# bit-current/DistributedTraining

Measured on AMD Instinct MI355X. Metric: tokens/sec (whole node, all miners), GPT-2-small local-SGD, higher is better.
Workload: dtype bf16; 1 GPU; model=gpt2-small, global_batch=1024, seq_len=64, parallelism=local_sgd_dp1, merge_every=25, optimizer=fused AdamW (lr 5e-4, reference config)

## Files before the change

### distributedtraining_amd/ops/__init__.py

```python

from __future__ import annotations

import math
from typing import Optional

import torch
import torch.nn.functional as F

from . import droprng
from .backend import require_ext, use_hip

__all__ = [
    "layer_norm", "rms_norm", "gelu", "swiglu", "causal_attention",
    "qkv_attention", "linear", "mlp_gelu", "add_layer_norm",
    "add_rms_norm",
    "cross_entropy_loss", "lm_head_ce", "lm_head_loss",
    "embedding_fwd",
    "decode_attention", "rope", "adamw_step", "delta_sub", "axpy_",
    "weighted_merge",
    "grad_merge_weights", "has_nan", "l2norm",
    "quantize_blockwise_int8", "dequantize_blockwise_int8",
    "dropout", "rng_tick",
]

# ... 22 lines not shown
        if dy2.stride(-1) != 1:
            dy2 = dy2.contiguous()
        dx = dy2.mm(w).view(ctx.xshape)
        m = require_ext()
        if _USE_BGRADB and ctx.has_b and ctx.wgrad is not None:
            try:
                db = m.lt_wgrad_bgradb(dy2, x2, ctx.wgrad)
                return dx, None, db
            except RuntimeError:
                pass
        if ctx.wgrad is not None:
            ctx.wgrad.addmm_(dy2.t(), x2)
            dw = None
        else:
            dw = dy2.t().mm(x2)
        db = (_grad_out(m.colsum(dy2), ctx.bgrad, w.dtype)
              if ctx.has_b else None)
        return dx, dw, db


def linear(x: torch.Tensor, w: torch.Tensor,
           b: Optional[torch.Tensor] = None) -> torch.Tensor:
    if use_hip(x):
        rows = x.numel() // x.shape[-1]
        if rows <= 4 and not torch.is_grad_enabled() and _gemv_wins(rows, w):
            x2 = x.reshape(rows, x.shape[-1])
            if not x2.is_contiguous():
                x2 = x2.contiguous()
            y = require_ext().gemv(
                x2, w, b if b is not None
                else torch.empty(0, dtype=w.dtype, device=w.device))
# ... 22 lines not shown
        y = torch.addmm(b2, h, w2.t())
        ctx.save_for_backward(x2, w1, w2, h, aux)
        ctx.xshape = x.shape
        ctx.w1grad = getattr(w1, "main_grad", None)
        ctx.w2grad = getattr(w2, "main_grad", None)
        ctx.b2grad = getattr(b2, "main_grad", None)
        return y.view(*x.shape[:-1], w2.shape[0])

    @staticmethod
    def backward(ctx, dy):
        m = require_ext()
        x2, w1, w2, h, aux = ctx.saved_tensors
        dy2 = dy.reshape(-1, dy.shape[-1])
        if dy2.stride(-1) != 1:
            dy2 = dy2.contiguous()
        db2 = _grad_out(m.colsum(dy2), ctx.b2grad, w2.dtype)
        if ctx.w2grad is not None:
            ctx.w2grad.addmm_(dy2.t(), h)
            dw2 = None
        else:
            dw2 = dy2.t().mm(h)
        dh_pre, db1 = m.lt_dgrad_dgelu_bgrad(dy2, w2, aux)
        if ctx.w1grad is not None:
            ctx.w1grad.addmm_(dh_pre.t(), x2)
            dw1 = None
        else:
            dw1 = dh_pre.t().mm(x2)
        dx = dh_pre.mm(w1).view(ctx.xshape)
        return dx, dw1, db1, dw2, db2


def mlp_gelu(x: torch.Tensor, w1: torch.Tensor, b1: torch.Tensor,
             w2: torch.Tensor, b2: torch.Tensor) -> torch.Tensor:
    if use_hip(x):
        rows = x.numel() // x.shape[-1]
        if rows <= 4 and not torch.is_grad_enabled():
            return linear(gelu(linear(x, w1, b1)), w2, b2)
        key = (rows, w1.shape[0], w1.shape[1])
        if _lt_fused_shape_ok.get(key, True):
            try:
                out = _FusedMLPFn.apply(x, w1, b1, w2, b2)
                _lt_fused_shape_ok[key] = True
                return out
            except RuntimeError as e:
                import logging
                logging.getLogger(__name__).warning(
                    "hipBLASLt epilogue MLP unavailable at M,N,K=%s (%s); "
                    "composed path", key, e)
                _lt_fused_shape_ok[key] = False
        return linear(gelu(linear(x, w1, b1)), w2, b2)
    return F.linear(F.gelu(F.linear(x, w1, b1), approximate="tanh"), w2, b2)


def _empty_like0(t):
    return t.new_empty(0)


def _rng0(t: torch.Tensor) -> torch.Tensor:
    return droprng.counter(t.device)


def _grad_out(fp32_grad, main_grad, dtype):
    if main_grad is not None:
        require_ext().accum_f32_into_bf16(main_grad, fp32_grad)
        return None
    return fp32_grad.to(dtype)


def _cpu_drop(t: torch.Tensor, p: float, site: int) -> torch.Tensor:
    keep = droprng.elem_keep_mask(t.numel(), droprng.value(t.device), site, p)
    mask = torch.from_numpy(keep.astype("float32")).reshape(t.shape)
    return t * (mask * droprng.inv_keep(p)).to(t.dtype)


def _norm_fwd(x2, res, w, b, eps, site, p):
    m = require_ext()
    if b is None:
        y, rstd, s = m.rmsnorm_fwd(x2, res, w, eps, _rng0(x2), site, p)
        return y, (rstd,), s
    y, mean, rstd, s = m.layernorm_fwd(x2, res, w, b, eps, _rng0(x2), site, p)
    return y, (mean, rstd), s


def _norm_bwd(dy, ds, x2, w, stats, site, p):
    m = require_ext()
    if len(stats) == 1:
        dx, dw32, dres = m.rmsnorm_bwd(dy, ds, x2, w, *stats, _rng0(x2),
                                       site, p)
        return dx, dw32, None, dres
    return m.layernorm_bwd(dy, ds, x2, w, *stats, _rng0(x2), site, p)


class _NormFn(torch.autograd.Function):
    @staticmethod
    def forward(ctx, x, w, b, eps):
        x2 = x.contiguous()
        y, stats, _ = _norm_fwd(x2.view(-1, x2.shape[-1]), _empty_like0(x2),
                                w, b, eps, 0, 0.0)
        ctx.save_for_backward(x2, w, *stats)
        ctx.wg = getattr(w, "main_grad", None)
        ctx.bg = getattr(b, "main_grad", None)
        return y.view_as(x2)

    @staticmethod
    def backward(ctx, dy):
        x, w, *stats = ctx.saved_tensors
        N = x.shape[-1]
        dx, dw32, db32, _ = _norm_bwd(dy.contiguous().view(-1, N),
                                      _empty_like0(x), x.view(-1, N), w,
                                      stats, 0, 0.0)
        return (dx.view_as(x), _grad_out(dw32, ctx.wg, w.dtype),
                None if db32 is None else _grad_out(db32, ctx.bg, w.dtype),
                None)


def layer_norm(x: torch.Tensor, w: torch.Tensor, b: torch.Tensor,
               eps: float = 1e-5) -> torch.Tensor:
    if use_hip(x):
        return _NormFn.apply(x, w, b, eps)
    return F.layer_norm(x, (x.shape[-1],), w, b, eps)


class _AddNormFn(torch.autograd.Function):

    @staticmethod
    def forward(ctx, x, res, w, b, eps, p_drop, site):
        x2 = x.contiguous().view(-1, x.shape[-1])
        r2 = res.contiguous().view(-1, x.shape[-1])
# ... 1 lines not shown
        ctx.save_for_backward(s, w, *stats)
        ctx.shape = x.shape
        ctx.drop = (p_drop, site)
        ctx.wg = getattr(w, "main_grad", None)
        ctx.bg = getattr(b, "main_grad", None)
        return s.view(x.shape), y.view(x.shape)

    @staticmethod
    def backward(ctx, ds, dy):
        s, w, *stats = ctx.saved_tensors
        p_drop, site = ctx.drop
        N = s.shape[-1]
        ds2 = (ds.contiguous().view(-1, N) if ds is not None
               else _empty_like0(s))
        dx, dw32, db32, dres = _norm_bwd(dy.contiguous().view(-1, N), ds2, s,
                                         w, stats, site, p_drop)
        dx = dx.view(ctx.shape)
        dr = dres.view(ctx.shape) if p_drop > 0.0 else dx
        return (dx, dr, _grad_out(dw32, ctx.wg, w.dtype),
                None if db32 is None else _grad_out(db32, ctx.bg, w.dtype),
                None, None, None)


def add_layer_norm(x: torch.Tensor, res: torch.Tensor, w: torch.Tensor,
                   b: torch.Tensor, eps: float = 1e-5, p_drop: float = 0.0,
                   site: int = 0):
    if use_hip(x):
        return _AddNormFn.apply(x, res, w, b, eps, p_drop, site)
    if p_drop > 0.0:
        res = _cpu_drop(res, p_drop, site)
    s = x + res
    return s, F.layer_norm(s, (s.shape[-1],), w, b, eps)


def add_rms_norm(x: torch.Tensor, res: torch.Tensor, w: torch.Tensor,
# ... 696 lines not shown
```

### distributedtraining_amd/ops/hip/bindings.cpp

```cpp
#include <torch/extension.h>
#include <ATen/hip/HIPContext.h>

#include <algorithm>
#include <atomic>
#include <vector>

#include "dta_kernels.h"

namespace {

using torch::Tensor;

inline hipStream_t stream() {
  return at::hip::getCurrentHIPStream().stream();
}
inline const bf16_t* bfp(const Tensor& t) {
  return reinterpret_cast<const bf16_t*>(t.data_ptr());
}
inline bf16_t* bfp_mut(Tensor& t) {
  return reinterpret_cast<bf16_t*>(t.data_ptr());
}

void check_bf16(const Tensor& t, const char* name) {
  TORCH_CHECK(t.is_cuda(), name, " must be on GPU");
// ... 6 lines not shown
  TORCH_CHECK(t.is_contiguous(), name, " must be contiguous");
}

DropParams drop_params(const Tensor& rng, int64_t site, double p) {
  DropParams d;
  if (p > 0.0) {
    TORCH_CHECK(p < 1.0, "dropout p must be < 1");
    TORCH_CHECK(rng.numel() == 1 && rng.scalar_type() == torch::kInt64 &&
                    rng.is_cuda(), "rng must be an int64 [1] GPU counter");
    d.rng = reinterpret_cast<const unsigned long long*>(
        rng.data_ptr<int64_t>());
    d.site = (unsigned long long)site;
    dta_drop_quantize(p, d);
  }
  return d;
}

int norm_cols(const Tensor& x, int max_cols, const char* what) {
  check_bf16(x, "x");
  TORCH_CHECK(x.size(1) % 8 == 0, "cols must be a multiple of 8");
  TORCH_CHECK(x.size(1) <= max_cols, what, " supports cols <= ", max_cols,
              " (register-resident row)");
  return int(x.size(1));
}

std::vector<Tensor> norm_fwd(Tensor x, Tensor res, Tensor w, const Tensor* b,
                             double eps, Tensor rng, int64_t site, double p) {
  const int cols = norm_cols(x, DTA_NORM_FWD_MAX_COLS, "norm forward");
  check_bf16(w, "w");
  if (b) check_bf16(*b, "b");
// ... 6 lines not shown
  auto y = torch::empty_like(x);
  auto sum = has_res ? torch::empty_like(x) : torch::empty({0}, x.options());
  Tensor mean = b ? torch::empty({rows}, f32) : Tensor();
  auto rstd = torch::empty({rows}, f32);
  launch_norm_fwd({bfp(x), has_res ? bfp(res) : nullptr,
                   has_res ? bfp_mut(sum) : nullptr, bfp(w),
                   b ? bfp(*b) : nullptr, bfp_mut(y),
                   b ? mean.data_ptr<float>() : nullptr,
                   rstd.data_ptr<float>(), rows, cols, float(eps), drop, !b},
                  stream());
  return {y, mean, rstd, sum};
}

std::vector<Tensor> norm_bwd(Tensor dy, Tensor ds, Tensor x, Tensor w,
                             const Tensor* mean, Tensor rstd, Tensor rng,
                             int64_t site, double p) {
  const int cols = norm_cols(x, DTA_NORM_BWD_MAX_COLS, "norm backward");
  check_bf16(dy, "dy"); check_bf16(w, "w");
  const int64_t rows = x.size(0);
  const bool has_ds = ds.numel() > 0;
  if (has_ds) check_bf16(ds, "ds");
  const DropParams drop = drop_params(rng, site, p);
  auto dx = torch::empty_like(x);
  auto dres = drop.thr16 ? torch::empty_like(x)
                         : torch::empty({0}, x.options());
  const auto f32 = x.options().dtype(torch::kFloat32);
  auto dw32 = torch::zeros({cols}, f32);
  Tensor db32 = mean ? torch::zeros({cols}, f32) : Tensor();
  const int stripes = dta_norm_bwd_stripes(rows, cols);
  auto part = torch::empty({mean ? 2 : 1, stripes, cols}, f32);
  launch_norm_bwd({bfp(dy), has_ds ? bfp(ds) : nullptr, bfp(x), bfp(w),
                   mean ? mean->data_ptr<float>() : nullptr,
                   rstd.data_ptr<float>(), bfp_mut(dx),
                   drop.thr16 ? bfp_mut(dres) : nullptr,
                   dw32.data_ptr<float>(),
                   mean ? db32.data_ptr<float>() : nullptr,
                   part[0].data_ptr<float>(),
                   mean ? part[1].data_ptr<float>() : nullptr, stripes, rows,
                   cols, drop, !mean},
                  stream());
  return {dx, dw32, db32, dres};
}

std::vector<Tensor> layernorm_fwd(Tensor x, Tensor res, Tensor w, Tensor b,
                                  double eps, Tensor rng, int64_t site,
                                  double p) {
  return norm_fwd(x, res, w, &b, eps, rng, site, p);
}
std::vector<Tensor> layernorm_bwd(Tensor dy, Tensor ds, Tensor x, Tensor w,
                                  Tensor mean, Tensor rstd, Tensor rng,
                                  int64_t site, double p) {
  return norm_bwd(dy, ds, x, w, &mean, rstd, rng, site, p);
}
std::vector<Tensor> rmsnorm_fwd(Tensor x, Tensor res, Tensor w, double eps,
                                Tensor rng, int64_t site, double p) {
  auto o = norm_fwd(x, res, w, nullptr, eps, rng, site, p);
  return {o[0], o[2], o[3]};
}
std::vector<Tensor> rmsnorm_bwd(Tensor dy, Tensor ds, Tensor x, Tensor w,
                                Tensor rstd, Tensor rng, int64_t site,
                                double p) {
  auto o = norm_bwd(dy, ds, x, w, nullptr, rstd, rng, site, p);
  return {o[0], o[1], o[3]};
}

Tensor gelu_fwd(Tensor x) {
  auto y = torch::empty_like(x);
  if (x.scalar_type() == torch::kBFloat16) {
    check_bf16(x, "x");
    launch_gelu_fwd(bfp(x), bfp_mut(y), x.numel(), stream());
  } else {
    check_f32(x, "x");
    launch_gelu_fwd_f32(x.data_ptr<float>(), y.data_ptr<float>(), x.numel(),
                        stream());
  }
  return y;
}
// ... 79 lines not shown
  bf16_t* outp = out_bf16.numel() ? bfp_mut(out_bf16) : nullptr;
  const float* bcp = bc.numel() ? bc.data_ptr<float>() : nullptr;
  launch_adamw(master.data_ptr<float>(), grad.data_ptr(), gb,
               m.data_ptr<float>(), v.data_ptr<float>(), outp, int(step),
               bcp, float(lr), beta1, beta2, float(eps), float(wd),
               master.numel(), stream());
}

void adamw_tick(Tensor t, Tensor bc, double beta1, double beta2) {
  TORCH_CHECK(t.scalar_type() == torch::kInt32 && t.is_cuda(), "t int32 gpu");
  check_f32(bc, "bc");
  launch_adamw_tick(t.data_ptr<int>(), bc.data_ptr<float>(), beta1, beta2,
                    stream());
}

Tensor colsum(Tensor x) {
  check_bf16(x, "x");
  TORCH_CHECK(x.dim() == 2 && x.size(1) % 8 == 0,
              "x must be [rows, cols] with cols % 8 == 0");
  const int64_t rows = x.size(0);
  const int cols = int(x.size(1));
  const int stripes = dta_colred_stripes(rows, cols);
  auto f32 = x.options().dtype(torch::kFloat32);
  auto part = torch::empty({stripes, cols}, f32);
  auto out = torch::zeros({cols}, f32);
  launch_colsum(bfp(x), part.data_ptr<float>(), out.data_ptr<float>(), rows,
                cols, stripes, stream());
  return out;
}

void weighted_merge(Tensor base, Tensor deltas, Tensor W, Tensor offsets,
                    Tensor out) {
  check_f32(base, "base"); check_f32(deltas, "deltas"); check_f32(out, "out");
  auto Wc = W.to(base.device(), torch::kFloat32).contiguous();
  auto offs = offsets.to(base.device()).contiguous();
  const int n_models = int(deltas.size(0));
  const int n_segs = int(offsets.numel() - 1);
  launch_weighted_merge(base.data_ptr<float>(), deltas.data_ptr<float>(),
                        Wc.data_ptr<float>(), offs.data_ptr<int64_t>(),
                        n_models, n_segs, base.numel(),
                        out.data_ptr<float>(), stream());
}

// ... 342 lines not shown
  const int dim = int(dy.size(-1));
  const int seq = int(ids.size(-1));
  const int64_t n_tok = ids.numel();
  auto f32 = dy.options().dtype(torch::kFloat32);
  auto dwte = torch::zeros({vocab, dim}, f32);
  auto dwpe = npos ? torch::zeros({npos, dim}, f32) : torch::zeros({0}, f32);
  launch_embedding_bwd(bfp(dy), ids.data_ptr<int64_t>(),
                       dwte.data_ptr<float>(), nullptr, n_tok, seq, dim,
                       false, stream());
  if (npos) {
    const int64_t B = n_tok / seq;
    const int pcols = seq * dim;
    TORCH_CHECK(pcols % 8 == 0, "seq*dim must be a multiple of 8");
    const int stripes = dta_colred_stripes(B, pcols);
    auto part = torch::empty({stripes, pcols}, f32);
    launch_colsum(bfp(dy), part.data_ptr<float>(), dwpe.data_ptr<float>(),
                  B, pcols, stripes, stream());
  }
  return {dwte, dwpe};
}

Tensor gemv(Tensor x, Tensor w, Tensor bias) {
  check_bf16(x, "x"); check_bf16(w, "w");
  TORCH_CHECK(x.dim() == 2 && w.dim() == 2 && x.size(1) == w.size(1),
              "x [M,K], w [N,K]");
  const int M = int(x.size(0));
  TORCH_CHECK(M >= 1 && M <= 4, "gemv is for M <= 4");
  const int64_t N = w.size(0);
  const int K = int(x.size(1));
  TORCH_CHECK(K % 8 == 0, "gemv needs K % 8 == 0 (16 B row alignment)");
  const bf16_t* bp = nullptr;
  if (bias.numel()) {
// ... 205 lines not shown
}
Tensor mfma_selftest_32(Tensor A, Tensor B) {
  check_bf16(A, "A"); check_bf16(B, "B");
  auto D = torch::zeros({32, 32}, A.options().dtype(torch::kFloat32));
  launch_mfma_probe_32(bfp(A), bfp(B), D.data_ptr<float>(), stream());
  return D;
}

}

void register_lt_fused(pybind11::module& m);

PYBIND11_MODULE(TORCH_EXTENSION_NAME, m) {
  register_lt_fused(m);
  m.def("layernorm_fwd", &layernorm_fwd);
  m.def("layernorm_bwd", &layernorm_bwd);
  m.def("rmsnorm_fwd", &rmsnorm_fwd);
  m.def("rmsnorm_bwd", &rmsnorm_bwd);
  m.def("gelu_fwd", &gelu_fwd);
  m.def("gelu_bwd", &gelu_bwd);
  m.def("swiglu_fwd", &swiglu_fwd);
  m.def("swiglu_bwd", &swiglu_bwd);
  m.def("dropout_apply", &dropout_apply);
  m.def("rng_tick", &rng_tick);
  m.def("accum_f32_into_bf16", &accum_f32_into_bf16);
  m.def("delta_sub", &delta_sub);
  m.def("axpy", &axpy);
  m.def("has_nan", &has_nan);
  m.def("l2norm_sq", &l2norm_sq);
  m.def("adamw_step", &adamw_step);
  m.def("adamw_tick", &adamw_tick);
  m.def("colsum", &colsum);
  m.def("weighted_merge", &weighted_merge);
  m.def("grad_merge_weights", &grad_merge_weights);
  m.def("weighted_merge_packed", &weighted_merge_packed);
  m.def("grad_merge_weights_packed", &grad_merge_weights_packed);
  m.def("axpy_packed", &axpy_packed);
  m.def("quantize_int8", &quantize_int8);
  m.def("ce_fwd", &ce_fwd);
  m.def("ce_bwd", &ce_bwd);
  m.def("ce_fwd_bwd", &ce_fwd_bwd, pybind11::arg("logits"),
        pybind11::arg("targets"), pybind11::arg("ignore_index"),
        pybind11::arg("inv_count_dev"), pybind11::arg("max_rows") = 0,
        pybind11::arg("lds_row") = false);
  m.def("ce_chunk", &ce_chunk);
  m.def("ce_finalize", &ce_finalize);
  m.def("head_loss_fwd", &head_loss_fwd);
// ... 17 lines not shown
```

### distributedtraining_amd/ops/hip/dta_kernels.h

```cpp
#pragma once

#include <hip/hip_runtime.h>
#include <cmath>
#include <cstdint>
#include <cstdlib>

using bf16_t = unsigned short;

struct DropParams {
  const unsigned long long* rng = nullptr;
  unsigned long long site = 0;
  unsigned int thr16 = 0;
  float inv_keep = 1.0f;
};
inline void dta_drop_quantize(double p, DropParams& d) {
  const double full = 65536.0;
  d.thr16 = (unsigned int)std::fmin(std::ceil(p * full), full - 1.0);
  d.inv_keep = float(full / (full - double(d.thr16)));
}

void launch_gelu_fwd(const bf16_t* x, bf16_t* y, int64_t n, hipStream_t s);
void launch_gelu_bwd(const bf16_t* dy, const bf16_t* x, bf16_t* dx, int64_t n,
                     hipStream_t s);
void launch_gelu_fwd_f32(const float* x, float* y, int64_t n, hipStream_t s);
// ... 9 lines not shown
void launch_accum_f32_bf16(bf16_t* dst, const float* src, int64_t n,
                           hipStream_t s);

void launch_delta_sub(const float* w, const float* base, float* out,
                      int64_t n, hipStream_t s);
void launch_axpy(float* w, const float* x, float alpha, int64_t n,
                 hipStream_t s);
void launch_nan_any(const float* x, int64_t n, int* flag, hipStream_t s);
void launch_l2norm_sq(const float* x, int64_t n, float* out, hipStream_t s);
void launch_adamw(float* master, const void* grad, bool grad_is_bf16,
                  float* m, float* v, bf16_t* out_bf16, int step,
                  const float* bc_p, float lr, double beta1, double beta2,
                  float eps, float wd, int64_t n, hipStream_t s);
void launch_adamw_tick(int* t, float* bc, double beta1, double beta2,
                       hipStream_t s);
void launch_colsum(const bf16_t* x, float* part, float* out, int64_t rows,
                   int cols, int stripes, hipStream_t s);
struct ColRedCfg { int threads; int gx; int stripes; };
inline ColRedCfg dta_colred_cfg(int64_t rows, int cols) {
  const int lanes = cols / 8;
  const int gx = (lanes + 255) / 256;
  int threads = ((lanes + gx - 1) / gx + 63) / 64 * 64;
  if (threads < 64) threads = 64;
  int64_t st = (1024 * 256) / (int64_t(gx) * threads);
  const int64_t mx = (rows + 31) / 32;
  if (st > mx) st = mx;
  if (st < 1) st = 1;
  return ColRedCfg{threads, gx, int(st)};
}
inline int dta_colred_stripes(int64_t rows, int cols) {
  return dta_colred_cfg(rows, cols).stripes;
}

void launch_weighted_merge(const float* base, const float* deltas,
                           const float* W,
                           const int64_t* offsets, int n_models, int n_segs,
                           int64_t P, float* out, hipStream_t s);
void launch_grad_merge_weights(const void* g, bool g_is_bf16,
                               const float* base, const float* deltas,
                               const float* merged, const int64_t* chunks,
                               int n_models, int n_chunks, int64_t P,
                               float* grad_w,
                               int n_segs, hipStream_t s);
enum DeltaKind { DELTA_F32 = 0, DELTA_BF16 = 1, DELTA_I8 = 2 };
struct PackedView {
  const void* data;
// ... 47 lines not shown
  bf16_t* sum_out;
  const bf16_t *w, *b;
  bf16_t* y;
  float *mean, *rstd;
  int64_t rows;
  int cols;
  float eps;
  DropParams drop;
  bool rms;
};
struct NormBwdArgs {
  const bf16_t *dy, *ds, *x, *w;
  const float *mean, *rstd;
  bf16_t *dx, *dres;
  float *dw, *db, *pdw, *pdb;
  int stripes;
  int64_t rows;
  int cols;
  DropParams drop;
  bool rms;
};
void launch_norm_fwd(const NormFwdArgs& a, hipStream_t s);
void launch_norm_bwd(const NormBwdArgs& a, hipStream_t s);

void launch_ce_fwd(const bf16_t* logits, const int64_t* targets,
                   int64_t rows, int64_t vocab, int64_t ignore_index,
                   float* lse, float* loss_sum, int* count, hipStream_t s);
void launch_ce_bwd(const bf16_t* logits, const int64_t* targets,
                   const float* lse, float scale, const float* scale_p,
                   int64_t ignore_index, int64_t v0, bool nt,
// ... 106 lines not shown
```

### distributedtraining_amd/ops/hip/elementwise.hip

```cpp
#include "dta_common.h"
#include "dta_kernels.h"

namespace {

constexpr float GELU_C = 0.7978845608028654f;
constexpr float GELU_A = 0.044715f;

DEV float gelu_f(float x) {
  float u = GELU_C * (x + GELU_A * x * x * x);
  return 0.5f * x * (1.0f + fast_tanh(u));
}
DEV float gelu_df(float x) {
  float x2 = x * x;
  float u = GELU_C * x * (1.0f + GELU_A * x2);
  float t = fast_tanh(u);
  float sech2 = 1.0f - t * t;
  return 0.5f * (1.0f + t) + 0.5f * x * sech2 * GELU_C * (1.0f + 3.0f * GELU_A * x2);
}
DEV float silu_f(float x) { return x / (1.0f + fast_exp(-x)); }
DEV float silu_df(float x) {
  float s = 1.0f / (1.0f + fast_exp(-x));
  return s * (1.0f + x * (1.0f - s));
}

template <float (*F)(float)>
__global__ void map_bf16_k(const ushort* __restrict__ x, ushort* __restrict__ y,
                           int64_t n) {
  int64_t i = (int64_t(blockIdx.x) * blockDim.x + threadIdx.x) * 16;
  const int64_t stride = int64_t(gridDim.x) * blockDim.x * 16;
  for (; i + 16 <= n; i += stride) {
    s16x8 va = *reinterpret_cast<const s16x8*>(x + i);
    s16x8 vb = *reinterpret_cast<const s16x8*>(x + i + 8);
// ... 191 lines not shown
  const int c8 = (blockIdx.x * blockDim.x + threadIdx.x) * 8;
  if (c8 >= cols) return;
  const int64_t r0 = (rows * blockIdx.y) / gridDim.y;
  const int64_t r1 = (rows * (blockIdx.y + 1)) / gridDim.y;
  float acc[8] = {0.f, 0.f, 0.f, 0.f, 0.f, 0.f, 0.f, 0.f};
  for (int64_t r = r0; r < r1; ++r) {
    s16x8 vx = *reinterpret_cast<const s16x8*>(x + r * int64_t(cols) + c8);
#pragma unroll
    for (int j = 0; j < 8; ++j) acc[j] += bf2f(ushort(vx[j]));
  }
  float* p = part + int64_t(blockIdx.y) * cols + c8;
#pragma unroll
  for (int j = 0; j < 8; ++j) p[j] = acc[j];
}

__global__ void colsum_reduce_k(const float* __restrict__ part,
                                float* __restrict__ out, int stripes,
                                int cols) {
  const int c4 = (blockIdx.x * blockDim.x + threadIdx.x) * 4;
  if (c4 >= cols) return;
  const int s0 = (stripes * blockIdx.y) / gridDim.y;
  const int s1 = (stripes * (blockIdx.y + 1)) / gridDim.y;
  f32x4 acc = {0.f, 0.f, 0.f, 0.f};
  for (int s_ = s0; s_ < s1; ++s_)
    acc += *reinterpret_cast<const f32x4*>(part + int64_t(s_) * cols + c4);
#pragma unroll
  for (int j = 0; j < 4; ++j) atomicAdd(out + c4 + j, acc[j]);
}

__global__ void dropout_k(const ushort* __restrict__ x,
                          ushort* __restrict__ y, int64_t n,
                          const unsigned long long* __restrict__ rng,
                          unsigned long long site, unsigned int thr16,
                          float inv_keep) {
  const uint64_t s1 = rng_site_seed(rng, site);
  int64_t i = (int64_t(blockIdx.x) * blockDim.x + threadIdx.x) * 8;
  const int64_t stride = int64_t(gridDim.x) * blockDim.x * 8;
  for (; i + 8 <= n; i += stride) {
    s16x8 vx = *reinterpret_cast<const s16x8*>(x + i);
    const uint64_t h0 = rng_elem_hash(s1, uint64_t(i >> 2));
    const uint64_t h1 = rng_elem_hash(s1, uint64_t((i >> 2) + 1));
    s16x8 o;
// ... 70 lines not shown
  LAUNCH_EW(delta_sub_k, n, w, base, out, n);
}
void launch_axpy(float* w, const float* x, float alpha, int64_t n,
                 hipStream_t s) {
  LAUNCH_EW(axpy_k, n, w, x, alpha, n);
}
void launch_nan_any(const float* x, int64_t n, int* flag, hipStream_t s) {
  LAUNCH_EW(nan_any_k, n, x, n, flag);
}
void launch_l2norm_sq(const float* x, int64_t n, float* out, hipStream_t s) {
  LAUNCH_EW(l2norm_sq_k, n, x, n, out);
}
void launch_f32_to_bf16(const float* x, bf16_t* y, int64_t n, hipStream_t s) {
  LAUNCH_EW(f32_to_bf16_k, n, x, y, n);
}
void launch_colsum(const bf16_t* x, float* part, float* out, int64_t rows,
                   int cols, int stripes, hipStream_t s) {
  const ColRedCfg cfg = dta_colred_cfg(rows, cols);
  dim3 g1(cfg.gx, unsigned(stripes));
  colsum_part_k<<<g1, cfg.threads, 0, s>>>(x, part, rows, cols);
  const int g2 = (cols / 4 + 255) / 256;
  const int ry = stripes < 32 ? stripes : 32;
  colsum_reduce_k<<<dim3(g2, ry), 256, 0, s>>>(part, out, stripes, cols);
}
void launch_dropout(const bf16_t* x, bf16_t* y, int64_t n,
                    const DropParams& d, hipStream_t s) {
  LAUNCH_EW(dropout_k, n, x, y, n, d.rng, d.site, d.thr16, d.inv_keep);
}
void launch_rng_tick(unsigned long long* ctr, hipStream_t s) {
  rng_tick_k<<<1, 1, 0, s>>>(ctr);
}
void launch_accum_f32_bf16(bf16_t* dst, const float* src, int64_t n,
                           hipStream_t s) {
  LAUNCH_EW(accum_f32_bf16_k, n, dst, src, n);
}
```

### distributedtraining_amd/ops/hip/norms.hip

```cpp
#include "dta_common.h"
#include "dta_kernels.h"

#include <cstdio>
#include <type_traits>

namespace {

constexpr int ROW_WAVES = 4;

template <int ITERS, bool RMS, bool RES, bool DROP>
__global__ void norm_fwd_k(const ushort* __restrict__ x,
                           const ushort* __restrict__ res,
                           ushort* __restrict__ sum_out,
                           const ushort* __restrict__ w,
                           const ushort* __restrict__ b,
                           ushort* __restrict__ y, float* __restrict__ mean,
                           float* __restrict__ rstd, int64_t rows, int cols,
                           float eps,
                           const unsigned long long* __restrict__ rng,
                           unsigned long long site, unsigned int thr16,
                           float inv_keep) {
  const int lane = threadIdx.x & 63, wid = threadIdx.x >> 6;
  const int nchunk = cols >> 3;
  const uint64_t s1d = DROP ? rng_site_seed(rng, site) : 0;
// ... 234 lines not shown
      const float dyv = bf2f(ushort(dv[j]));
      dw_acc[j] = fmaf(dyv, (bf2f(ushort(xv[j])) - mu) * rs, dw_acc[j]);
      db_acc[j] += dyv;
    }
  }
  float* pw = pdw + int64_t(blockIdx.y) * cols + c8;
#pragma unroll
  for (int j = 0; j < 8; ++j) pw[j] = dw_acc[j];
  if (!RMS) {
    float* pb = pdb + int64_t(blockIdx.y) * cols + c8;
#pragma unroll
    for (int j = 0; j < 8; ++j) pb[j] = db_acc[j];
  }
}

__global__ void dwdb_reduce_k(const float* __restrict__ pdw,
                              const float* __restrict__ pdb,
                              float* __restrict__ dw, float* __restrict__ db,
                              int stripes, int cols) {
  const int c4 = (blockIdx.x * blockDim.x + threadIdx.x) * 4;
  if (c4 >= cols) return;
  const int s0 = (stripes * blockIdx.y) / gridDim.y;
  const int s1 = (stripes * (blockIdx.y + 1)) / gridDim.y;
  f32x4 aw = {0.f, 0.f, 0.f, 0.f};
  f32x4 ab = {0.f, 0.f, 0.f, 0.f};
  for (int s_ = s0; s_ < s1; ++s_) {
    aw += *reinterpret_cast<const f32x4*>(pdw + int64_t(s_) * cols + c4);
    if (pdb)
      ab += *reinterpret_cast<const f32x4*>(pdb + int64_t(s_) * cols + c4);
  }
#pragma unroll
  for (int j = 0; j < 4; ++j) {
    atomicAdd(dw + c4 + j, aw[j]);
    if (pdb) atomicAdd(db + c4 + j, ab[j]);
  }
}

constexpr int NORM_ITERS[] = {1, 2, 3, 4, 6, 8, 16};
constexpr int N_NORM_ITERS = sizeof(NORM_ITERS) / sizeof(int);
constexpr int ITER_COLS = WAVE * 8;
static_assert(NORM_ITERS[N_NORM_ITERS - 1] * ITER_COLS == DTA_NORM_FWD_MAX_COLS &&
              NORM_ITERS[N_NORM_ITERS - 2] * ITER_COLS == DTA_NORM_BWD_MAX_COLS);

template <int MAXC, int K = 0, class F>
void with_iters(int cols, F&& f) {
  if constexpr (K < N_NORM_ITERS && NORM_ITERS[K] * ITER_COLS <= MAXC) {
    if (cols <= NORM_ITERS[K] * ITER_COLS)
      f(std::integral_constant<int, NORM_ITERS[K]>{});
    else
      with_iters<MAXC, K + 1>(cols, f);
  } else {
    fprintf(stderr, "norm kernels: cols=%d beyond the limit %d\n", cols, MAXC);
// ... 31 lines not shown
  const DropParams& d = a.drop;
  with_flags([&](auto RMS, auto DS, auto DROP, auto FDW) {
    with_iters<DTA_NORM_BWD_MAX_COLS>(a.cols, [&](auto I) {
      norm_bwd_dx_k<I, RMS, DS, DROP, FDW><<<grid, 64 * ROW_WAVES, 0, s>>>(
          a.dy, a.ds, a.x, a.w, a.mean, a.rstd, a.dx, a.dres,
          FDW ? a.pdw : nullptr, FDW ? a.pdb : nullptr, a.rows, a.cols,
          d.rng, d.site, d.thr16, d.inv_keep);
    });
    if (!FDW) {
      const ColRedCfg cfg = dta_colred_cfg(a.rows, a.cols);
      norm_bwd_dwdb_part_k<RMS>
          <<<dim3(cfg.gx, unsigned(a.stripes)), cfg.threads, 0, s>>>(
              a.dy, a.x, a.mean, a.rstd, a.pdw, a.pdb, a.rows, a.cols);
    }
  }, a.rms, a.ds != nullptr, d.thr16 != 0, dta_norm_fused_dwdb(a.cols));
  const int g3 = (a.cols / 4 + 255) / 256;
  const int ry =
      a.stripes < 32 ? a.stripes : (a.stripes > 1024 ? 256 : 32);
  dwdb_reduce_k<<<dim3(g3, ry), 256, 0, s>>>(a.pdw, a.pdb, a.dw, a.db,
                                             a.stripes, a.cols);
}
```

Measured before the change: 911,300 tokens/s.

## Fuse bias-grad reductions into main_grad accumulation and add GELU-bwd colsum MLP path

Replaces the atomic-based column-reduction finishers (colsum and norm dw/db) with a single shared finish kernel. It reduces the partials in-block and accumulates straight into the bf16 main_grad, removing the separate zeros memset, atomics and accum_f32_into_bf16 launches. Adds a fused GELU-backward+bias-colsum kernel and a composed MLP autograd node for when the hipBLASLt epilogue path is unavailable. This cuts kernel launches and memory passes in the backward pass, but changes reduction order and adds complexity.

Result: faster. 926,700 tokens/s, median of 6 (+1.7%).

```diff
diff --git a/distributedtraining_amd/ops/__init__.py b/distributedtraining_amd/ops/__init__.py
--- a/distributedtraining_amd/ops/__init__.py
+++ b/distributedtraining_amd/ops/__init__.py
@@ -60,7 +60,7 @@
             dw = None
         else:
             dw = dy2.t().mm(x2)
-        db = (_grad_out(m.colsum(dy2), ctx.bgrad, w.dtype)
+        db = (_cast_grad(m.colsum(dy2, ctx.bgrad), w.dtype)
               if ctx.has_b else None)
         return dx, dw, db
 
@@ -113,7 +113,7 @@
         dy2 = dy.reshape(-1, dy.shape[-1])
         if dy2.stride(-1) != 1:
             dy2 = dy2.contiguous()
-        db2 = _grad_out(m.colsum(dy2), ctx.b2grad, w2.dtype)
+        db2 = _cast_grad(m.colsum(dy2, ctx.b2grad), w2.dtype)
         if ctx.w2grad is not None:
             ctx.w2grad.addmm_(dy2.t(), h)
             dw2 = None
@@ -127,6 +127,56 @@
             dw1 = dh_pre.t().mm(x2)
         dx = dh_pre.mm(w1).view(ctx.xshape)
         return dx, dw1, db1, dw2, db2
+
+
+_MLP_NODE = _os.environ.get("DTA_MLP_NODE", "1") != "0"
+
+
+def mlp_node_enable(on: bool) -> bool:
+    global _MLP_NODE
+    prev, _MLP_NODE = _MLP_NODE, bool(on)
+    return prev
+
+
+class _MLPGeluFn(torch.autograd.Function):
+
+    @staticmethod
+    def forward(ctx, x, w1, b1, w2, b2):
+        m = require_ext()
+        x2 = x.reshape(-1, x.shape[-1])
+        pre = torch.addmm(b1, x2, w1.t())
+        h = m.gelu_fwd(pre)
+        y = torch.addmm(b2, h, w2.t())
+        ctx.save_for_backward(x2, w1, w2, pre, h)
+        ctx.xshape = x.shape
+        ctx.grads = tuple(getattr(t, "main_grad", None)
+                          for t in (w1, b1, w2, b2))
+        return y.view(*x.shape[:-1], w2.shape[0])
+
+    @staticmethod
+    def backward(ctx, dy):
+        m = require_ext()
+        x2, w1, w2, pre, h = ctx.saved_tensors
+        w1g, b1g, w2g, b2g = ctx.grads
+        dy2 = dy.reshape(-1, dy.shape[-1])
+        if dy2.stride(-1) != 1:
+            dy2 = dy2.contiguous()
+        dh = dy2.mm(w2)
+        if w2g is not None:
+            w2g.addmm_(dy2.t(), h)
+            dw2 = None
+        else:
+            dw2 = dy2.t().mm(h)
+        db2 = _cast_grad(m.colsum(dy2, b2g), w2.dtype)
+        dh_pre, db1 = m.gelu_bwd_colsum(dh, pre, b1g)
+        del dh
+        dx = dh_pre.mm(w1).view(ctx.xshape)
+        if w1g is not None:
+            w1g.addmm_(dh_pre.t(), x2)
+            dw1 = None
+        else:
+            dw1 = dh_pre.t().mm(x2)
+        return dx, dw1, _cast_grad(db1, w1.dtype), dw2, db2
 
 
 def mlp_gelu(x: torch.Tensor, w1: torch.Tensor, b1: torch.Tensor,
@@ -147,6 +197,9 @@
                     "hipBLASLt epilogue MLP unavailable at M,N,K=%s (%s); "
                     "composed path", key, e)
                 _lt_fused_shape_ok[key] = False
+        if _MLP_NODE and all(t.dtype == torch.bfloat16
+                             for t in (x, w1, b1, w2, b2)):
+            return _MLPGeluFn.apply(x, w1, b1, w2, b2)
         return linear(gelu(linear(x, w1, b1)), w2, b2)
     return F.linear(F.gelu(F.linear(x, w1, b1), approximate="tanh"), w2, b2)
 
@@ -164,6 +217,10 @@
         require_ext().accum_f32_into_bf16(main_grad, fp32_grad)
         return None
     return fp32_grad.to(dtype)
+
+
+def _cast_grad(fp32_grad, dtype):
+    return None if fp32_grad is None else fp32_grad.to(dtype)
 
 
 def _cpu_drop(t: torch.Tensor, p: float, site: int) -> torch.Tensor:
@@ -181,13 +238,13 @@
     return y, (mean, rstd), s
 
 
-def _norm_bwd(dy, ds, x2, w, stats, site, p):
+def _norm_bwd(dy, ds, x2, w, stats, site, p, wg=None, bg=None):
     m = require_ext()
     if len(stats) == 1:
         dx, dw32, dres = m.rmsnorm_bwd(dy, ds, x2, w, *stats, _rng0(x2),
-                                       site, p)
+                                       site, p, wg)
         return dx, dw32, None, dres
-    return m.layernorm_bwd(dy, ds, x2, w, *stats, _rng0(x2), site, p)
+    return m.layernorm_bwd(dy, ds, x2, w, *stats, _rng0(x2), site, p, wg, bg)
 
 
 class _NormFn(torch.autograd.Function):
@@ -207,10 +264,9 @@
         N = x.shape[-1]
         dx, dw32, db32, _ = _norm_bwd(dy.contiguous().view(-1, N),
                                       _empty_like0(x), x.view(-1, N), w,
-                                      stats, 0, 0.0)
-        return (dx.view_as(x), _grad_out(dw32, ctx.wg, w.dtype),
-                None if db32 is None else _grad_out(db32, ctx.bg, w.dtype),
-                None)
+                                      stats, 0, 0.0, ctx.wg, ctx.bg)
+        return (dx.view_as(x), _cast_grad(dw32, w.dtype),
+                _cast_grad(db32, w.dtype), None)
 
 
 def layer_norm(x: torch.Tensor, w: torch.Tensor, b: torch.Tensor,
@@ -242,11 +298,11 @@
         ds2 = (ds.contiguous().view(-1, N) if ds is not None
                else _empty_like0(s))
         dx, dw32, db32, dres = _norm_bwd(dy.contiguous().view(-1, N), ds2, s,
-                                         w, stats, site, p_drop)
+                                         w, stats, site, p_drop, ctx.wg,
+                                         ctx.bg)
         dx = dx.view(ctx.shape)
         dr = dres.view(ctx.shape) if p_drop > 0.0 else dx
-        return (dx, dr, _grad_out(dw32, ctx.wg, w.dtype),
-                None if db32 is None else _grad_out(db32, ctx.bg, w.dtype),
+        return (dx, dr, _cast_grad(dw32, w.dtype), _cast_grad(db32, w.dtype),
                 None, None, None)
 
 
diff --git a/distributedtraining_amd/ops/hip/bindings.cpp b/distributedtraining_amd/ops/hip/bindings.cpp
--- a/distributedtraining_amd/ops/hip/bindings.cpp
+++ b/distributedtraining_amd/ops/hip/bindings.cpp
@@ -44,6 +44,14 @@
     dta_drop_quantize(p, d);
   }
   return d;
+}
+
+using OptTensor = c10::optional<Tensor>;
+bf16_t* grad_dst(OptTensor& d, int64_t cols, const char* name) {
+  if (!d.has_value() || !d->defined()) return nullptr;
+  check_bf16(*d, name);
+  TORCH_CHECK(d->numel() == cols, name, " must have cols elements");
+  return bfp_mut(*d);
 }
 
 int norm_cols(const Tensor& x, int max_cols, const char* what) {
@@ -80,7 +88,8 @@
 
 std::vector<Tensor> norm_bwd(Tensor dy, Tensor ds, Tensor x, Tensor w,
                              const Tensor* mean, Tensor rstd, Tensor rng,
-                             int64_t site, double p) {
+                             int64_t site, double p, OptTensor dw_dst,
+                             OptTensor db_dst) {
   const int cols = norm_cols(x, DTA_NORM_BWD_MAX_COLS, "norm backward");
   check_bf16(dy, "dy"); check_bf16(w, "w");
   const int64_t rows = x.size(0);
@@ -91,18 +100,21 @@
   auto dres = drop.thr16 ? torch::empty_like(x)
                          : torch::empty({0}, x.options());
   const auto f32 = x.options().dtype(torch::kFloat32);
-  auto dw32 = torch::zeros({cols}, f32);
-  Tensor db32 = mean ? torch::zeros({cols}, f32) : Tensor();
+  bf16_t* dwd = grad_dst(dw_dst, cols, "dw_dst");
+  bf16_t* dbd = mean ? grad_dst(db_dst, cols, "db_dst") : nullptr;
+  Tensor dw32 = dwd ? Tensor() : torch::empty({cols}, f32);
+  Tensor db32 = (mean && !dbd) ? torch::empty({cols}, f32) : Tensor();
   const int stripes = dta_norm_bwd_stripes(rows, cols);
   auto part = torch::empty({mean ? 2 : 1, stripes, cols}, f32);
   launch_norm_bwd({bfp(dy), has_ds ? bfp(ds) : nullptr, bfp(x), bfp(w),
                    mean ? mean->data_ptr<float>() : nullptr,
                    rstd.data_ptr<float>(), bfp_mut(dx),
                    drop.thr16 ? bfp_mut(dres) : nullptr,
-                   dw32.data_ptr<float>(),
-                   mean ? db32.data_ptr<float>() : nullptr,
+                   dwd ? nullptr : dw32.data_ptr<float>(),
+                   db32.defined() ? db32.data_ptr<float>() : nullptr,
                    part[0].data_ptr<float>(),
-                   mean ? part[1].data_ptr<float>() : nullptr, stripes, rows,
+                   mean ? part[1].data_ptr<float>() : nullptr, dwd, dbd,
+                   stripes, rows,
                    cols, drop, !mean},
                   stream());
   return {dx, dw32, db32, dres};
@@ -115,8 +127,9 @@
 }
 std::vector<Tensor> layernorm_bwd(Tensor dy, Tensor ds, Tensor x, Tensor w,
                                   Tensor mean, Tensor rstd, Tensor rng,
-                                  int64_t site, double p) {
-  return norm_bwd(dy, ds, x, w, &mean, rstd, rng, site, p);
+                                  int64_t site, double p, OptTensor dw_dst,
+                                  OptTensor db_dst) {
+  return norm_bwd(dy, ds, x, w, &mean, rstd, rng, site, p, dw_dst, db_dst);
 }
 std::vector<Tensor> rmsnorm_fwd(Tensor x, Tensor res, Tensor w, double eps,
                                 Tensor rng, int64_t site, double p) {
@@ -125,8 +138,9 @@
 }
 std::vector<Tensor> rmsnorm_bwd(Tensor dy, Tensor ds, Tensor x, Tensor w,
                                 Tensor rstd, Tensor rng, int64_t site,
-                                double p) {
-  auto o = norm_bwd(dy, ds, x, w, nullptr, rstd, rng, site, p);
+                                double p, OptTensor dw_dst) {
+  auto o = norm_bwd(dy, ds, x, w, nullptr, rstd, rng, site, p, dw_dst,
+                    c10::nullopt);
   return {o[0], o[1], o[3]};
 }
 
@@ -236,19 +250,46 @@
                     stream());
 }
 
-Tensor colsum(Tensor x) {
+Tensor colsum(Tensor x, OptTensor dst) {
   check_bf16(x, "x");
-  TORCH_CHECK(x.dim() == 2 && x.size(1) % 8 == 0,
-              "x must be [rows, cols] with cols % 8 == 0");
+  TORCH_CHECK(x.dim() == 2 && x.size(1) >= 1, "x must be [rows, cols]");
   const int64_t rows = x.size(0);
   const int cols = int(x.size(1));
   const int stripes = dta_colred_stripes(rows, cols);
   auto f32 = x.options().dtype(torch::kFloat32);
+  auto part = torch::empty({stripes, dta_colred_ld(cols)}, f32);
+  bf16_t* d = grad_dst(dst, cols, "dst");
+  Tensor out = d ? Tensor() : torch::empty({cols}, f32);
+  launch_colsum(bfp(x), part.data_ptr<float>(),
+                d ? nullptr : out.data_ptr<float>(), d, rows, cols, stripes,
+                stream());
+  return out;
+}
+
+std::vector<Tensor> gelu_bwd_colsum(Tensor dy, Tensor x, OptTensor db_dst,
+                                    int64_t stripes_arg) {
+  check_bf16(x, "x"); check_bf16(dy, "dy");
+  TORCH_CHECK(x.dim() == 2 && dy.sizes() == x.sizes(),
+              "dy, x must be [rows, cols]");
+  const int64_t rows = x.size(0);
+  const int cols = int(x.size(1));
+  if (cols % 8 != 0) {
+    auto dx = gelu_bwd(dy, x);
+    return {dx, colsum(dx, db_dst)};
+  }
+  const int stripes =
+      stripes_arg > 0 ? int(std::min<int64_t>(stripes_arg, 65535))
+                      : dta_gelu_colsum_stripes(rows, cols);
+  auto f32 = x.options().dtype(torch::kFloat32);
+  auto dx = torch::empty_like(x);
   auto part = torch::empty({stripes, cols}, f32);
-  auto out = torch::zeros({cols}, f32);
-  launch_colsum(bfp(x), part.data_ptr<float>(), out.data_ptr<float>(), rows,
-                cols, stripes, stream());
-  return out;
+  bf16_t* d = grad_dst(db_dst, cols, "db_dst");
+  Tensor out = d ? Tensor() : torch::empty({cols}, f32);
+  launch_gelu_bwd_colsum(bfp(dy), bfp(x), bfp_mut(dx),
+                         part.data_ptr<float>(),
+                         d ? nullptr : out.data_ptr<float>(), d, rows, cols,
+                         stripes, stream());
+  return {dx, out};
 }
 
 void weighted_merge(Tensor base, Tensor deltas, Tensor W, Tensor offsets,
@@ -621,8 +662,9 @@
     TORCH_CHECK(pcols % 8 == 0, "seq*dim must be a multiple of 8");
     const int stripes = dta_colred_stripes(B, pcols);
     auto part = torch::empty({stripes, pcols}, f32);
+    TORCH_CHECK(seq <= npos, "seq must be <= npos");
     launch_colsum(bfp(dy), part.data_ptr<float>(), dwpe.data_ptr<float>(),
-                  B, pcols, stripes, stream());
+                  nullptr, B, pcols, stripes, stream());
   }
   return {dwte, dwpe};
 }
@@ -858,11 +900,19 @@
 PYBIND11_MODULE(TORCH_EXTENSION_NAME, m) {
   register_lt_fused(m);
   m.def("layernorm_fwd", &layernorm_fwd);
-  m.def("layernorm_bwd", &layernorm_bwd);
+  namespace py = pybind11;
+  m.def("layernorm_bwd", &layernorm_bwd, py::arg("dy"), py::arg("ds"),
+        py::arg("x"), py::arg("w"), py::arg("mean"), py::arg("rstd"),
+        py::arg("rng"), py::arg("site"), py::arg("p"),
+        py::arg("dw_dst") = py::none(), py::arg("db_dst") = py::none());
   m.def("rmsnorm_fwd", &rmsnorm_fwd);
-  m.def("rmsnorm_bwd", &rmsnorm_bwd);
+  m.def("rmsnorm_bwd", &rmsnorm_bwd, py::arg("dy"), py::arg("ds"),
+        py::arg("x"), py::arg("w"), py::arg("rstd"), py::arg("rng"),
+        py::arg("site"), py::arg("p"), py::arg("dw_dst") = py::none());
   m.def("gelu_fwd", &gelu_fwd);
   m.def("gelu_bwd", &gelu_bwd);
+  m.def("gelu_bwd_colsum", &gelu_bwd_colsum, py::arg("dy"), py::arg("x"),
+        py::arg("db_dst") = py::none(), py::arg("stripes") = 0);
   m.def("swiglu_fwd", &swiglu_fwd);
   m.def("swiglu_bwd", &swiglu_bwd);
   m.def("dropout_apply", &dropout_apply);
@@ -874,7 +924,7 @@
   m.def("l2norm_sq", &l2norm_sq);
   m.def("adamw_step", &adamw_step);
   m.def("adamw_tick", &adamw_tick);
-  m.def("colsum", &colsum);
+  m.def("colsum", &colsum, py::arg("x"), py::arg("dst") = py::none());
   m.def("weighted_merge", &weighted_merge);
   m.def("grad_merge_weights", &grad_merge_weights);
   m.def("weighted_merge_packed", &weighted_merge_packed);
diff --git a/distributedtraining_amd/ops/hip/dta_kernels.h b/distributedtraining_amd/ops/hip/dta_kernels.h
--- a/distributedtraining_amd/ops/hip/dta_kernels.h
+++ b/distributedtraining_amd/ops/hip/dta_kernels.h
@@ -47,12 +47,24 @@
                   float eps, float wd, int64_t n, hipStream_t s);
 void launch_adamw_tick(int* t, float* bc, double beta1, double beta2,
                        hipStream_t s);
-void launch_colsum(const bf16_t* x, float* part, float* out, int64_t rows,
-                   int cols, int stripes, hipStream_t s);
+struct ColFinishArgs {
+  const float *p0, *p1;
+  float *out0, *out1;
+  bf16_t *dst0, *dst1;
+  int stripes, cols, ld;
+};
+void launch_colred_finish(const ColFinishArgs& a, hipStream_t s);
+inline int dta_colred_ld(int cols) { return (cols + 3) / 4 * 4; }
+void launch_colsum(const bf16_t* x, float* part, float* out, bf16_t* dst,
+                   int64_t rows, int cols, int stripes, hipStream_t s);
+void launch_gelu_bwd_colsum(const bf16_t* dy, const bf16_t* x, bf16_t* dx,
+                            float* part, float* out, bf16_t* dst,
+                            int64_t rows, int cols, int stripes,
+                            hipStream_t s);
 struct ColRedCfg { int threads; int gx; int stripes; };
 inline ColRedCfg dta_colred_cfg(int64_t rows, int cols) {
   const int lanes = cols / 8;
-  const int gx = (lanes + 255) / 256;
+  const int gx = lanes > 0 ? (lanes + 255) / 256 : 1;
   int threads = ((lanes + gx - 1) / gx + 63) / 64 * 64;
   if (threads < 64) threads = 64;
   int64_t st = (1024 * 256) / (int64_t(gx) * threads);
@@ -63,6 +75,11 @@
 }
 inline int dta_colred_stripes(int64_t rows, int cols) {
   return dta_colred_cfg(rows, cols).stripes;
+}
+inline int dta_gelu_colsum_stripes(int64_t rows, int cols) {
+  const int64_t st = int64_t(dta_colred_stripes(rows, cols)) * 3 / 2;
+  const int64_t mx = (rows + 31) / 32;
+  return int(st > mx ? (mx > 0 ? mx : 1) : st);
 }
 
 void launch_weighted_merge(const float* base, const float* deltas,
@@ -140,6 +157,7 @@
   const float *mean, *rstd;
   bf16_t *dx, *dres;
   float *dw, *db, *pdw, *pdb;
+  bf16_t *dw_dst, *db_dst;
   int stripes;
   int64_t rows;
   int cols;
diff --git a/distributedtraining_amd/ops/hip/elementwise.hip b/distributedtraining_amd/ops/hip/elementwise.hip
--- a/distributedtraining_amd/ops/hip/elementwise.hip
+++ b/distributedtraining_amd/ops/hip/elementwise.hip
@@ -11,11 +11,14 @@
   return 0.5f * x * (1.0f + fast_tanh(u));
 }
 DEV float gelu_df(float x) {
+#pragma clang fp contract(off)
   float x2 = x * x;
-  float u = GELU_C * x * (1.0f + GELU_A * x2);
+  float u = (GELU_C * x) * (1.0f + GELU_A * x2);
   float t = fast_tanh(u);
-  float sech2 = 1.0f - t * t;
-  return 0.5f * (1.0f + t) + 0.5f * x * sech2 * GELU_C * (1.0f + 3.0f * GELU_A * x2);
+  float sech2 = __builtin_fmaf(-t, t, 1.0f);
+  float q = __builtin_fmaf(3.0f * GELU_A, x2, 1.0f);
+  float p = (((0.5f * x) * sech2) * GELU_C) * q;
+  return __builtin_fmaf(1.0f + t, 0.5f, p);
 }
 DEV float silu_f(float x) { return x / (1.0f + fast_exp(-x)); }
 DEV float silu_df(float x) {
@@ -237,18 +240,139 @@
   for (int j = 0; j < 8; ++j) p[j] = acc[j];
 }
 
-__global__ void colsum_reduce_k(const float* __restrict__ part,
-                                float* __restrict__ out, int stripes,
-                                int cols) {
-  const int c4 = (blockIdx.x * blockDim.x + threadIdx.x) * 4;
-  if (c4 >= cols) return;
-  const int s0 = (stripes * blockIdx.y) / gridDim.y;
-  const int s1 = (stripes * (blockIdx.y + 1)) / gridDim.y;
-  f32x4 acc = {0.f, 0.f, 0.f, 0.f};
-  for (int s_ = s0; s_ < s1; ++s_)
-    acc += *reinterpret_cast<const f32x4*>(part + int64_t(s_) * cols + c4);
-#pragma unroll
-  for (int j = 0; j < 4; ++j) atomicAdd(out + c4 + j, acc[j]);
+__global__ void colsum_part_any_k(const ushort* __restrict__ x,
+                                  float* __restrict__ part, int64_t rows,
+                                  int cols, int ld) {
+  const int c = blockIdx.x * blockDim.x + threadIdx.x;
+  if (c >= ld) return;
+  const int64_t r0 = (rows * blockIdx.y) / gridDim.y;
+  const int64_t r1 = (rows * (blockIdx.y + 1)) / gridDim.y;
+  float acc = 0.f;
+  if (c < cols)
+    for (int64_t r = r0; r < r1; ++r) acc += bf2f(x[r * int64_t(cols) + c]);
+  part[int64_t(blockIdx.y) * ld + c] = acc;
+}
+
+__global__ void gelu_bwd_colsum_k(const ushort* __restrict__ dy,
+                                  const ushort* __restrict__ x,
+                                  ushort* __restrict__ dx,
+                                  float* __restrict__ part, int64_t rows,
+                                  int cols) {
+  const int c8 = (blockIdx.x * blockDim.x + threadIdx.x) * 8;
+  if (c8 >= cols) return;
+  const int64_t r0 = (rows * blockIdx.y) / gridDim.y;
+  const int64_t r1 = (rows * (blockIdx.y + 1)) / gridDim.y;
+  float acc[8] = {0.f, 0.f, 0.f, 0.f, 0.f, 0.f, 0.f, 0.f};
+  int64_t r = r0;
+  for (; r + 2 <= r1; r += 2) {
+    const int64_t ia = r * int64_t(cols) + c8, ib = ia + cols;
+    s16x8 da = *reinterpret_cast<const s16x8*>(dy + ia);
+    s16x8 db = *reinterpret_cast<const s16x8*>(dy + ib);
+    s16x8 xa = *reinterpret_cast<const s16x8*>(x + ia);
+    s16x8 xb = *reinterpret_cast<const s16x8*>(x + ib);
+    s16x8 oa, ob;
+#pragma unroll
+    for (int j = 0; j < 8; ++j) {
+      oa[j] = f2bf(bf2f(ushort(da[j])) * gelu_df(bf2f(ushort(xa[j]))));
+      ob[j] = f2bf(bf2f(ushort(db[j])) * gelu_df(bf2f(ushort(xb[j]))));
+    }
+    *reinterpret_cast<s16x8*>(dx + ia) = oa;
+    *reinterpret_cast<s16x8*>(dx + ib) = ob;
+#pragma unroll
+    for (int j = 0; j < 8; ++j) {
+      acc[j] += bf2f(ushort(oa[j]));
+      acc[j] += bf2f(ushort(ob[j]));
+    }
+  }
+  if (r < r1) {
+    const int64_t ia = r * int64_t(cols) + c8;
+    s16x8 da = *reinterpret_cast<const s16x8*>(dy + ia);
+    s16x8 xa = *reinterpret_cast<const s16x8*>(x + ia);
+    s16x8 oa;
+#pragma unroll
+    for (int j = 0; j < 8; ++j) {
+      oa[j] = f2bf(bf2f(ushort(da[j])) * gelu_df(bf2f(ushort(xa[j]))));
+      acc[j] += bf2f(ushort(oa[j]));
+    }
+    *reinterpret_cast<s16x8*>(dx + ia) = oa;
+  }
+  float* p = part + int64_t(blockIdx.y) * cols + c8;
+#pragma unroll
+  for (int j = 0; j < 8; ++j) p[j] = acc[j];
+}
+
+constexpr int FIN_THREADS = 256;
+constexpr int FIN_COLS = 8;
+constexpr int FIN_CL = FIN_COLS / 4;
+constexpr int FIN_SL = FIN_THREADS / FIN_CL;
+static_assert(FIN_CL == 2 && FIN_THREADS == 4 * WAVE,
+              "colred_finish_k's shuffle tree folds lanes 2..63 of 4 waves");
+
+DEV void finish_write(f32x4 v, float* out, ushort* dst, int c4, int cols) {
+  if (dst) {
+    ushort* d = dst + c4;
+    if (c4 + 4 <= cols && (reinterpret_cast<uintptr_t>(d) & 7) == 0) {
+      s16x4 o = *reinterpret_cast<const s16x4*>(d);
+#pragma unroll
+      for (int j = 0; j < 4; ++j) o[j] = f2bf(bf2f(ushort(o[j])) + v[j]);
+      *reinterpret_cast<s16x4*>(d) = o;
+    } else {
+#pragma unroll
+      for (int j = 0; j < 4; ++j)
+        if (c4 + j < cols) d[j] = f2bf(bf2f(d[j]) + v[j]);
+    }
+  } else if (c4 + 4 <= cols && (reinterpret_cast<uintptr_t>(out + c4) & 15) == 0) {
+    *reinterpret_cast<f32x4*>(out + c4) = v;
+  } else {
+#pragma unroll
+    for (int j = 0; j < 4; ++j)
+      if (c4 + j < cols) out[c4 + j] = v[j];
+  }
+}
+
+__global__ void __launch_bounds__(FIN_THREADS)
+colred_finish_k(const float* __restrict__ p0, const float* __restrict__ p1,
+                float* __restrict__ out0, float* __restrict__ out1,
+                ushort* __restrict__ dst0, ushort* __restrict__ dst1,
+                int stripes, int cols, int ld) {
+  __shared__ f32x4 lds[2][FIN_THREADS / WAVE][FIN_CL];
+  const int cl = threadIdx.x & (FIN_CL - 1), sl = threadIdx.x / FIN_CL;
+  const int wid = threadIdx.x / WAVE;
+  const int c4 = (blockIdx.x * FIN_CL + cl) * 4;
+  const bool live = c4 < ld;
+  f32x4 a0 = {0.f, 0.f, 0.f, 0.f}, a1 = {0.f, 0.f, 0.f, 0.f};
+  if (live) {
+    const float* q0 = p0 + c4;
+    const float* q1 = p1 ? p1 + c4 : nullptr;
+#pragma unroll 4
+    for (int s_ = sl; s_ < stripes; s_ += FIN_SL) {
+      a0 += *reinterpret_cast<const f32x4*>(q0 + int64_t(s_) * ld);
+      if (q1) a1 += *reinterpret_cast<const f32x4*>(q1 + int64_t(s_) * ld);
+    }
+  }
+#pragma unroll
+  for (int off = FIN_CL; off < WAVE; off <<= 1) {
+#pragma unroll
+    for (int j = 0; j < 4; ++j) {
+      a0[j] += __shfl_xor(a0[j], off);
+      a1[j] += __shfl_xor(a1[j], off);
+    }
+  }
+  if ((threadIdx.x & (WAVE - 1)) < FIN_CL) {
+    lds[0][wid][cl] = a0;
+    lds[1][wid][cl] = a1;
+  }
+  __syncthreads();
+  if (threadIdx.x < FIN_CL && live) {
+    f32x4 r0 = lds[0][0][cl], r1 = lds[1][0][cl];
+#pragma unroll
+    for (int w = 1; w < FIN_THREADS / WAVE; ++w) {
+      r0 += lds[0][w][cl];
+      r1 += lds[1][w][cl];
+    }
+    finish_write(r0, out0, dst0, c4, cols);
+    if (p1) finish_write(r1, out1, dst1, c4, cols);
+  }
 }
 
 __global__ void dropout_k(const ushort* __restrict__ x,
@@ -349,14 +473,35 @@
 void launch_f32_to_bf16(const float* x, bf16_t* y, int64_t n, hipStream_t s) {
   LAUNCH_EW(f32_to_bf16_k, n, x, y, n);
 }
-void launch_colsum(const bf16_t* x, float* part, float* out, int64_t rows,
-                   int cols, int stripes, hipStream_t s) {
+void launch_colred_finish(const ColFinishArgs& a, hipStream_t s) {
+  const int grid = (a.ld / 4 + FIN_CL - 1) / FIN_CL;
+  colred_finish_k<<<grid, FIN_THREADS, 0, s>>>(a.p0, a.p1, a.out0, a.out1,
+                                               a.dst0, a.dst1, a.stripes,
+                                               a.cols, a.ld);
+}
+void launch_colsum(const bf16_t* x, float* part, float* out, bf16_t* dst,
+                   int64_t rows, int cols, int stripes, hipStream_t s) {
+  const int ld = dta_colred_ld(cols);
+  if (cols % 8 == 0) {
+    const ColRedCfg cfg = dta_colred_cfg(rows, cols);
+    dim3 g1(cfg.gx, unsigned(stripes));
+    colsum_part_k<<<g1, cfg.threads, 0, s>>>(x, part, rows, cols);
+  } else {
+    dim3 g1((ld + 255) / 256, unsigned(stripes));
+    colsum_part_any_k<<<g1, 256, 0, s>>>(x, part, rows, cols, ld);
+  }
+  launch_colred_finish({part, nullptr, out, nullptr, dst, nullptr, stripes,
+                        cols, ld}, s);
+}
+void launch_gelu_bwd_colsum(const bf16_t* dy, const bf16_t* x, bf16_t* dx,
+                            float* part, float* out, bf16_t* dst,
+                            int64_t rows, int cols, int stripes,
+                            hipStream_t s) {
   const ColRedCfg cfg = dta_colred_cfg(rows, cols);
   dim3 g1(cfg.gx, unsigned(stripes));
-  colsum_part_k<<<g1, cfg.threads, 0, s>>>(x, part, rows, cols);
-  const int g2 = (cols / 4 + 255) / 256;
-  const int ry = stripes < 32 ? stripes : 32;
-  colsum_reduce_k<<<dim3(g2, ry), 256, 0, s>>>(part, out, stripes, cols);
+  gelu_bwd_colsum_k<<<g1, cfg.threads, 0, s>>>(dy, x, dx, part, rows, cols);
+  launch_colred_finish({part, nullptr, out, nullptr, dst, nullptr, stripes,
+                        cols, cols}, s);
 }
 void launch_dropout(const bf16_t* x, bf16_t* y, int64_t n,
                     const DropParams& d, hipStream_t s) {
diff --git a/distributedtraining_amd/ops/hip/norms.hip b/distributedtraining_amd/ops/hip/norms.hip
--- a/distributedtraining_amd/ops/hip/norms.hip
+++ b/distributedtraining_amd/ops/hip/norms.hip
@@ -272,28 +272,6 @@
   }
 }
 
-__global__ void dwdb_reduce_k(const float* __restrict__ pdw,
-                              const float* __restrict__ pdb,
-                              float* __restrict__ dw, float* __restrict__ db,
-                              int stripes, int cols) {
-  const int c4 = (blockIdx.x * blockDim.x + threadIdx.x) * 4;
-  if (c4 >= cols) return;
-  const int s0 = (stripes * blockIdx.y) / gridDim.y;
-  const int s1 = (stripes * (blockIdx.y + 1)) / gridDim.y;
-  f32x4 aw = {0.f, 0.f, 0.f, 0.f};
-  f32x4 ab = {0.f, 0.f, 0.f, 0.f};
-  for (int s_ = s0; s_ < s1; ++s_) {
-    aw += *reinterpret_cast<const f32x4*>(pdw + int64_t(s_) * cols + c4);
-    if (pdb)
-      ab += *reinterpret_cast<const f32x4*>(pdb + int64_t(s_) * cols + c4);
-  }
-#pragma unroll
-  for (int j = 0; j < 4; ++j) {
-    atomicAdd(dw + c4 + j, aw[j]);
-    if (pdb) atomicAdd(db + c4 + j, ab[j]);
-  }
-}
-
 constexpr int NORM_ITERS[] = {1, 2, 3, 4, 6, 8, 16};
 constexpr int N_NORM_ITERS = sizeof(NORM_ITERS) / sizeof(int);
 constexpr int ITER_COLS = WAVE * 8;
@@ -355,9 +333,6 @@
               a.dy, a.x, a.mean, a.rstd, a.pdw, a.pdb, a.rows, a.cols);
     }
   }, a.rms, a.ds != nullptr, d.thr16 != 0, dta_norm_fused_dwdb(a.cols));
-  const int g3 = (a.cols / 4 + 255) / 256;
-  const int ry =
-      a.stripes < 32 ? a.stripes : (a.stripes > 1024 ? 256 : 32);
-  dwdb_reduce_k<<<dim3(g3, ry), 256, 0, s>>>(a.pdw, a.pdb, a.dw, a.db,
-                                             a.stripes, a.cols);
-}
+  launch_colred_finish({a.pdw, a.pdb, a.dw, a.db, a.dw_dst, a.db_dst,
+                        a.stripes, a.cols, a.cols}, s);
+}
```
